# jacobwilliams/lbfgsb

Measured on NVIDIA B200. Metric: lbfgsb_iterations_per_s, higher is better.
Workload: dtype f64

## Files before the change

### lbfgsb_b200/csrc/engine.cu

```cuda
#include <cuda_runtime.h>
#include <dlfcn.h>
#include <stdarg.h>
#include <stdio.h>
#include <stdlib.h>
#include <string.h>

#include <mutex>
#include <string>
#include <unordered_set>
#include <vector>

#include "../../include/lbfgsb_b200.h"
#include "cauchy_walk.cuh"
#include "kernels_tma.cuh"
#include "cauchy_walk_dist.cuh"
#include "batch.cuh"
#include "host_print.h"
#include <algorithm>

static thread_local std::string g_last_error;
static void set_error(const char* fmt, ...) {
    char buf[512];
    va_list ap;
    va_start(ap, fmt);
// ... 199 lines not shown
        for (int q = 0; q < F_COUNT; ++q) { fam_ms[q] = 0; fam_calls[q] = 0; }
        if (st) stream = st;
        else { CK(cudaStreamCreateWithFlags(&stream, cudaStreamNonBlocking)); own_stream = true; }
        memset(&w, 0, sizeof w);
        w.n = n; w.m = m; w.off = offset;
        w.ldw = (n + 31) / 32 * 32;
        const size_t vb = (size_t)w.ldw * sizeof(T);
        if (!dalloc(&w.ws, vb * m) || !dalloc(&w.wy, vb * m)) return false;
        if (!dalloc(&w.z, vb) || !dalloc(&w.r, vb) || !dalloc(&w.d, vb) || !dalloc(&w.t, vb) || !dalloc(&w.xp, vb) || !dalloc(&w.gold, vb)) return false;
        if (!dalloc(&w.iwhere, (size_t)w.ldw * 4) || !dalloc(&w.state, (size_t)w.ldw)) return false;
        if (!dalloc(&w.part, sizeof(T) * LB_KMAX * LBFGSB_GRID) || !dalloc(&w.ipart, sizeof(i64) * LB_IMAX * LBFGSB_GRID)) return false;
        if (!dalloc(&w.part2, sizeof(T) * LB_KMAX * LBFGSB_GRID) || !dalloc(&w.ipart2, sizeof(i64) * LB_IMAX * LBFGSB_GRID)) return false;
        if (!dalloc(&s_dev, sizeof(DevState<T>)) || !dalloc(&pub_counter, 8) || !dalloc(&f_dev, sizeof(T))) return false;
        CK(cudaMemsetAsync(s_dev, 0, sizeof(DevState<T>), stream));
        CK(cudaMemsetAsync(pub_counter, 0, 8, stream));
        {
            i64 lim = (i64)1 << 28;
            if (R > 1) lim = (i64)1 << 26;
            if (const char* e = getenv("LBFGSB_B200_TIE_LIMIT")) lim = atoll(e);
            CK(cudaMemcpyAsync(&s_dev->tie_limit, &lim, sizeof lim, cudaMemcpyHostToDevice, stream));
        }
        CK(cudaMemsetAsync(w.ws, 0, vb * m, stream));
        CK(cudaMemsetAsync(w.wy, 0, vb * m, stream));
        w.s = s_dev;
        CK(cudaHostAlloc((void**)&s_host, sizeof(DevState<T>) + 64, cudaHostAllocMapped));
        memset(s_host, 0, sizeof(DevState<T>) + 64);
        pub_flag = (volatile unsigned long long*)((char*)s_host + ((sizeof(DevState<T>) + 7) / 8) * 8);
        CK(cudaMallocHost((void**)&ctl_host, sizeof(SortCtl)));
        header_bytes = offsetof(DevState<T>, sy);
        const i64 tile = (i64)LBFGSB_BLOCK * Real<T>::VEC * Real<T>::UNROLL;
        ntiles = (n + tile - 1) / tile;
        if (!dalloc(&tile_counts, sizeof(int) * (size_t)(ntiles + 1)) || !dalloc(&tile_offsets, sizeof(i64) * (size_t)(ntiles + 1))) return false;
        if (!dalloc(&rs_counts, sizeof(int) * 256 * LB_RS_GRID)) return false;
        typedef typename Real<T>::key_t K;
        memset(&wb, 0, sizeof wb);
        if (!dalloc(&wb.k0, sizeof(K) * (size_t)w.ldw) || !dalloc(&wb.k1, sizeof(K) * (size_t)w.ldw)) return false;
        if (!dalloc(&wb.v0, 4 * (size_t)w.ldw) || !dalloc(&wb.v1, 4 * (size_t)w.ldw)) return false;
        if (!dalloc(&wb.ctl, sizeof(SortCtl)) || !dalloc(&ctl_el, sizeof(SortCtl))) return false;
        i64 cap = n < (i64)(1 << 22) ? n : (i64)(1 << 22);
        cap = (cap + LB_WB - 1) / LB_WB * LB_WB;
        wb.cap = cap;
        const size_t cb = (size_t)cap * sizeof(T);
        if (!dalloc(&wb.wj, cb * 2 * m) || !dalloc(&wb.vj, cb * 2 * m)) return false;
        if (!dalloc(&wb.delta, cb) || !dalloc(&wb.zeta, cb) || !dalloc(&wb.omega, cb) || !dalloc(&wb.g2, cb) ||
            !dalloc(&wb.g1, cb) || !dalloc(&wb.f1a, cb) || !dalloc(&wb.f2a, cb)) return false;
        const i64 nblk = cap / LB_WB;
// ... 863 lines not shown
        i64 my_tie_limit = 0;
        if (ok && !write) ok = cudaMemcpy(&my_tie_limit, &s_dev->tie_limit, sizeof my_tie_limit, cudaMemcpyDeviceToHost) == cudaSuccess;
        const size_t CH = (size_t)64 << 20;
        void* stage = nullptr;
        if (ok && cudaMallocHost(&stage, CH) != cudaSuccess) { set_error("cudaMallocHost failed"); ok = false; }
        auto xfer = [&](void* dptr, size_t bytes) {
            for (size_t o = 0; ok && o < bytes; o += CH) {
                const size_t c = bytes - o < CH ? bytes - o : CH;
                if (write) {
                    ok = cudaMemcpy(stage, (char*)dptr + o, c, cudaMemcpyDeviceToHost) == cudaSuccess && fwrite(stage, 1, c, fp) == c;
                } else {
                    ok = fread(stage, 1, c, fp) == c && cudaMemcpy((char*)dptr + o, stage, c, cudaMemcpyHostToDevice) == cudaSuccess;
                }
            }
        };
        const size_t vb = (size_t)w.ldw * sizeof(T);
        xfer(s_dev, sizeof(DevState<T>));
        xfer(w.ws, vb * m); xfer(w.wy, vb * m);
        xfer(w.z, vb); xfer(w.r, vb); xfer(w.d, vb); xfer(w.t, vb); xfer(w.xp, vb); xfer(w.gold, vb);
        xfer(w.iwhere, (size_t)w.ldw * 4); xfer(w.state, (size_t)w.ldw);
        if (stage) cudaFreeHost(stage);
        if (ok && !write) ok = cudaMemcpy(&s_dev->tie_limit, &my_tie_limit, sizeof my_tie_limit, cudaMemcpyHostToDevice) == cudaSuccess;
        if (ok && !write) ok = cudaMemcpy(s_host, s_dev, header_bytes, cudaMemcpyDeviceToHost) == cudaSuccess;
        if (ok && !write) started = true;
        if (write && ok) ok = fflush(fp) == 0;
        if (fclose(fp) != 0) ok = false;
        if (write) {
            if (ok) ok = rename(tmp.c_str(), path) == 0;
            else remove(tmp.c_str());
        }
        if (!ok && g_last_error.empty()) set_error("checkpoint %s failed on %s", write ? "write" : "read", path);
        return ok;
    }

    bool active_hash(uint64_t* hash, i64* count) {
        begin(F_HASH); k_active_hash<T><<<LG>>>(w, offset); end(F_HASH);
        std::vector<i64> hp(2 * LBFGSB_GRID);
        CK(cudaMemcpyAsync(hp.data(), w.ipart, sizeof(i64) * 2 * LBFGSB_GRID, cudaMemcpyDeviceToHost, stream));
        CK(cudaStreamSynchronize(stream));
        uint64_t h = 0; i64 c = 0;
        for (int b = 0; b < LBFGSB_GRID; ++b) { h += (uint64_t)hp[b]; c += hp[LBFGSB_GRID + b]; }
        *hash = h; *count = c;
        return true;
    }
};

// ... 944 lines not shown
    if (!nccl_api()->ok) { set_error("libnccl.so.2 not found"); return nullptr; }
    ncclComm_t c = nullptr;
    ncclUniqueId id;
    memcpy(&id, id128, sizeof id);
    int rc = nccl_api()->CommInitRank(&c, world, id, rank);
    if (rc != 0) { set_error("ncclCommInitRank failed: %d", rc); return nullptr; }
    return c;
}
void lbfgsb_dev_nccl_destroy(void* comm) { if (comm && nccl_api()->ok) nccl_api()->CommDestroy((ncclComm_t)comm); }

int lbfgsb_dev_active_set_hash(lbfgsb_dev_t* h, uint64_t* hash, int64_t* count) {
    EngineBase* b = (EngineBase*)h;
    if (!b) return 1;
    i64 c = 0;
    bool ok = (b->real_kind == 8) ? ((Engine<double>*)b)->active_hash(hash, &c) : ((Engine<float>*)b)->active_hash(hash, &c);
    *count = c;
    return ok ? 0 : 1;
}
void* lbfgsb_dev_vector(lbfgsb_dev_t* h, int32_t which) {
    EngineBase* b = (EngineBase*)h;
    if (!b) return nullptr;
#define VSEL(E)                                                                                          \
    switch (which) { case 0: return E->w.z; case 1: return E->w.r; case 2: return E->w.d; case 3: return E->w.t; \
                     case 4: return E->w.xp; case 5: return E->w.ws; case 6: return E->w.wy; case 7: return E->w.iwhere; case 8: return E->w.gold; default: return nullptr; }
    if (b->real_kind == 8) { Engine<double>* e = (Engine<double>*)b; VSEL(e) }
    else { Engine<float>* e = (Engine<float>*)b; VSEL(e) }
}
int lbfgsb_dev_vector_copy(lbfgsb_dev_t* h, int32_t which, void* dst_dev, int64_t bytes) {
    void* src = lbfgsb_dev_vector(h, which);
    if (!src || !dst_dev || bytes < 0) return 1;
    EngineBase* b = (EngineBase*)h;
    const i64 ldw = (b->real_kind == 8) ? ((Engine<double>*)b)->w.ldw : ((Engine<float>*)b)->w.ldw;
    const i64 m = (b->real_kind == 8) ? ((Engine<double>*)b)->w.m : ((Engine<float>*)b)->w.m;
    const i64 cap = (which == 7) ? ldw * 4 : ((which == 5 || which == 6) ? m : 1) * ldw * (i64)b->real_kind;
    if (bytes > cap) { set_error("lbfgsb_dev_vector_copy: %lld bytes requested, vector %d holds %lld", (long long)bytes, (int)which, (long long)cap); return 1; }
    if (cudaDeviceSynchronize() != cudaSuccess) return 1;
    return cudaMemcpy(dst_dev, src, (size_t)bytes, cudaMemcpyDeviceToDevice) != cudaSuccess;
}
int lbfgsb_dev_exchange_mode(lbfgsb_dev_t* h) {
    EngineBase* b = (EngineBase*)h;
    if (!b) return -1;
    if (b->real_kind == 8) { Engine<double>* e = (Engine<double>*)b; return e->R <= 1 ? 0 : (e->p2p ? 2 : 1); }
    Engine<float>* e = (Engine<float>*)b; return e->R <= 1 ? 0 : (e->p2p ? 2 : 1);
}
int lbfgsb_dev_counters(lbfgsb_dev_t* h, int64_t* launches, int64_t* syncs) {
    EngineBase* b = (EngineBase*)h;
    if (!b) return 1;
    if (b->real_kind == 8) { *launches = ((Engine<double>*)b)->launches; *syncs = ((Engine<double>*)b)->syncs; }
    else { *launches = ((Engine<float>*)b)->launches; *syncs = ((Engine<float>*)b)->syncs; }
    return 0;
}
void lbfgsb_dev_profile(lbfgsb_dev_t* h, int32_t enable) {
    EngineBase* b = (EngineBase*)h;
    if (!b) return;
    if (b->real_kind == 8) ((Engine<double>*)b)->profile = enable != 0; else ((Engine<float>*)b)->profile = enable != 0;
}
void lbfgsb_dev_set_tie_limit(lbfgsb_dev_t* h, int64_t max_breakpoints) {
// ... 321 lines not shown
```

### lbfgsb_b200/csrc/kernels_dense.cuh

```cuda
#pragma once
#include "kernels_stream.cuh"

#define LB_SCALAR_THREADS 256

template <typename T>
struct Red {
    T rv[LB_KMAX];
    i64 iv[LB_IMAX];
};

enum { OP_SUM = 0, OP_MAX = 1, OP_MIN = 2, OP_ARGMIN = 3  };

struct SiteSpec {
    int nreal;
    int nint;
    int argmin_slot;
    int max_from, max_to;
    int min_from, min_to;
    int imin_from, imin_to;
    int imax_from, imax_to;
    int buf;
};

template <typename T>
// ... 348 lines not shown
        if (s->nbreak != 0 && !(s->dtm < s->bkmin)) {
            s->need_walk = 1; s->lazy_gcp = 0;
            for (int j = 0; j < col2; ++j) { s->p0[j] = s->p[j]; s->walkA[j] = zero; s->walkB[j] = zero; }
            s->walk_f1 = s->f1; s->walk_f2 = s->f2; s->walk_tlast = zero; s->walk_tprev2 = zero;
            s->walk_J = -1; s->walk_done = 0; s->walk_base = 0; s->walk_rcount = 0; s->walk_lcount = 0; s->walk_rem = 0;
            s->walk_cstart = 0; s->walk_fixn = 0; s->walk_closed = 0; s->tie_redo = 0; s->tie_round = 0;
            stop = 1;
        } else {
            if (s->dtm <= zero) s->dtm = zero;
            s->tsum = s->tsum + s->dtm;
            if (col > 0) dense::daxpy<T>(col2, s->dtm, s->p, s->c);
        }
    }
    stop = __shfl_sync(LB_FULL, stop, 0);
    if (stop) return;
    __syncwarp();
    if (fused_supported && col > 0 && s->cnstnd) {
        const int info = wdense::bmv<T>(m, ssy, swt, col, s->c, s->a);
        if (info == 0 && lane == 0) s->fuse_gf = 1;
    }
    __syncwarp();
}

template <typename T> __device__ inline void w_freev(DevState<T>* s, const Red<T>& red, i64 n_global, bool gf, bool have) {
    const int lane = threadIdx.x & 31;
    int need_a = 0;
    if (lane == 0) {
        if (s->fuse_gf == 1) s->lazy_z = 1;
        if (have) {
            s->nintol = s->nintol + s->nseg;
            s->nfree = red.iv[0];
            s->nenter = red.iv[1];
            s->nleave = red.iv[2];
            s->wrk = (s->nleave > 0) || (s->nenter > 0) || s->updatd;
            s->nact = n_global - s->nfree;
        }
        s->do_subspace = !(s->nfree == 0 || s->col == 0);
        s->do_formk = s->do_subspace && s->wrk;
        s->do_delta = s->do_formk && (s->nenter + s->nleave > 0);
        need_a = (!gf && s->do_subspace && !(!s->cnstnd && s->col > 0)) ? 1 : 0;
    }
    need_a = __shfl_sync(LB_FULL, need_a, 0);
    __syncwarp();
    if (need_a) {
        int info = wdense::bmv<T>(s->m, s->sy, s->wt, s->col, s->c, s->a);
        if (info != 0 && lane == 0) {
            ev_push<T>(s, EV_SUBSM_SINGULAR);
            reset_memory<T>(s);
            s->restart = 1; s->in_body = 0; s->do_subspace = 0; s->do_formk = 0; s->do_delta = 0;
        }
// ... 316 lines not shown
    if (!fused_supported || s->col <= 0 || !s->cnstnd || s->fuse_gf) return;
    stage_in<T>(ssy, s->sy, s->m * s->m); stage_in<T>(swt, s->wt, s->m * s->m);
    __syncthreads();
    if (threadIdx.x >= 32) return;
    const int info = wdense::bmv<T>(s->m, ssy, swt, s->col, s->c, s->a);
    if (info == 0 && (threadIdx.x & 31) == 0) s->fuse_gf = 2;
}

template <typename T>
__global__ void __launch_bounds__(LB_SCALAR_THREADS) s_freev(Wk<T> w, Dist<T> dist, i64 n_global, int phase) {
    __shared__ Red<T> red;
    DevState<T>* s = w.s;
    site_fetch<T>(w, dist);
    if (!s->go || !s->in_body) return;
    const bool gf = s->fuse_gf != 0;
    if (phase == 1 && !gf) return;
    if (phase == 0 && gf) {
        if (threadIdx.x == 0) { s->do_subspace = 1; s->do_formk = s->updatd; s->do_delta = 0; }
        return;
    }
    const int mode = s->cauchy_mode;
    if (mode != 1) site_reduce<T>(w, dist, site_freev(), &red);
    if (threadIdx.x >= 32) return;
    w_freev<T>(s, red, n_global, gf, mode != 1);
}

template <typename T>
__global__ void __launch_bounds__(LB_SCALAR_THREADS) s_formk_dense(Wk<T> w, Dist<T> dist, int mt, const T* delta, T* delta_sum) {
    __shared__ Red<T> red;
    DevState<T>* s = w.s;
    site_fetch<T>(w, dist);
    if (!s->go || !s->in_body || !s->do_subspace) return;
    const bool newrow = s->do_formk && s->updatd;
    if (newrow) site_reduce<T>(w, dist, site_formk(mt), &red);
    if (dist.R > 1 && s->do_delta) {
        if (dist.p2p) p2p_wait<T>(w, dist.p2p->dflag, dist.R, dist.dseq);
        const volatile T* dv = delta;
        for (int e = threadIdx.x; e < 6 * LB_MMAX * LB_MMAX; e += blockDim.x) {
            T acc = dv[e];
            for (int q = 1; q < dist.R; ++q) acc = acc + dv[(i64)q * (6 * LB_MMAX * LB_MMAX) + e];
            delta_sum[e] = acc;
        }
        __syncthreads();
        delta = delta_sum;
    }
    __shared__ T swn[4 * LB_MMAX * LB_MMAX], swn1[4 * LB_MMAX * LB_MMAX];
    const bool stage = s->do_formk != 0;
// ... 187 lines not shown
    if (upd) { stage_out<T>(s->sy, ssy, mm); stage_out<T>(s->ss, sss, mm); stage_out<T>(s->wt, swt, mm); }
    if (!cont) return;
    site_reduce<T>(w, dist, ms.sp[1], &red, ms.roff[1], ms.ioff[1]);
    if (threadIdx.x >= 32) return;
    w_cauchy<T>(s, red, mt, ssy, swt, 1);
    if (threadIdx.x != 0) return;
    if (!s->in_body) return;
    if (s->need_walk) { s->pause = PAUSE_WALK; return; }
    if (!s->fuse_gf) { s->pause = PAUSE_GCP_FREEV; return; }
    s->do_subspace = 1; s->do_formk = s->updatd; s->do_delta = 0;
}

template <typename T>
__global__ void __launch_bounds__(LB_SCALAR_THREADS) f_mid(Wk<T> w, Dist<T> dist, int mt, i64 n_global) {
    __shared__ Red<T> red;
    __shared__ T swn[4 * LB_MMAX * LB_MMAX], swn1[4 * LB_MMAX * LB_MMAX];
    __shared__ int cont;
    DevState<T>* s = w.s;
    const MSite ms = msite_mid(mt);
    site_fetch<T>(w, dist);
    if (!s->go || s->pause || !s->in_body) return;
    site_reduce<T>(w, dist, ms.sp[0], &red, ms.roff[0], ms.ioff[0]);
    if (threadIdx.x < 32) {
        w_freev<T>(s, red, n_global, true, true);
        if (threadIdx.x == 0) {
            cont = 1;
            if (!s->do_subspace) { s->pause = PAUSE_LSINIT; cont = 0; }
            else if (s->do_delta) { s->pause = PAUSE_DELTA; cont = 0; }
        }
    }
    __syncthreads();
    if (!cont) return;
    const bool newrow = s->do_formk && s->updatd;
    if (newrow) site_reduce<T>(w, dist, ms.sp[1], &red, ms.roff[1], ms.ioff[1]);
    const bool stage = s->do_formk != 0;
    const int m4 = 4 * s->m * s->m;
    stage_in<T>(swn, s->wn, m4);
    if (stage) stage_in<T>(swn1, s->wn1, m4);
    __syncthreads();
    if (threadIdx.x < 32) w_formk_dense<T>(s, red, mt, (const T*)nullptr, swn, swn1);
    __syncthreads();
    if (stage) { stage_out<T>(s->wn, swn, m4); stage_out<T>(s->wn1, swn1, m4); }
    if (!s->in_body) return;
    site_reduce<T>(w, dist, ms.sp[2], &red, ms.roff[2], ms.ioff[2]);
    if (threadIdx.x >= 32) return;
    w_subsm_dense<T>(s, red, mt, swn, 1);
}
// ... 22 lines not shown
```

### lbfgsb_b200/csrc/kernels_stream.cuh

```cuda
#pragma once
#include "common.cuh"

template <typename T>
struct Wk {
    i64 n, ldw;
    i64 off;
    int m;
    T *ws, *wy;
    T *z, *r, *d, *t, *xp;
    T* gold;
    int* iwhere;
    unsigned char* state;
    T* part;
    i64* ipart;
    T* part2;
    i64* ipart2;
    DevState<T>* s;
    T* x; const T* l; const T* u; const int* nbd; T* g;
    int bp_hint;
};

#define LB_SLOT(part, k) ((part) + (i64)(k) * LBFGSB_GRID)
#define LB_INF(T) ((T)INFINITY)
#define LB_I64MAX 0x7fffffffffffffffLL

template <typename T>
__global__ void __launch_bounds__(LBFGSB_BLOCK) k_errclb(Wk<T> w) {
    constexpr int VEC = Real<T>::VEC;
    i64 k6 = -1, k7 = -1;
    LB_FOR_TILES(T, w.n, base) {
        T l[VEC], u[VEC]; int nb[VEC];
        ldv<T>(w.l, base, w.n, l); ldv<T>(w.u, base, w.n, u); ldvi<T>(w.nbd, base, w.n, nb);
#pragma unroll
        for (int v = 0; v < VEC; ++v) {
            i64 i = base + v;
            if (i < w.n) {
                if (nb[v] < 0 || nb[v] > 3) k6 = i;
                if (nb[v] == 2 && l[v] > u[v]) k7 = i;
            }
        }
    }
    i64 m6 = k6, m7 = k7;
// ... 342 lines not shown
```

### lbfgsb_b200/csrc/kernels_tma.cuh

```cuda
#pragma once
#include "kernels_stream.cuh"
#include "tma_pipe.cuh"

template <typename T, int MT> struct SubT { static constexpr int v = (sizeof(T) * MT <= 80) ? 256 : 128; };

template <typename T> struct SpecializeFullHistory { static constexpr bool value = sizeof(T) == 4; };
template <bool B> struct BoolC { static constexpr bool value = B; };

#define LB_DYN_STAGES(dyn) (dyn)

template <typename T>
__device__ __forceinline__ void pipe_add_w(PipeSrc* ps, const Wk<T>& w, int head0, int count, unsigned slot) {
    int pj = head0;
    for (int j = 0; j < count; ++j) {
        pipe_add(ps, w.wy + (i64)pj * w.ldw, (int)sizeof(T), slot);
        pipe_add(ps, w.ws + (i64)pj * w.ldw, (int)sizeof(T), slot);
        pj = (pj + 1 == w.m) ? 0 : pj + 1;
    }
}

template <typename T, int MT>
__global__ void __launch_bounds__(LB_TMA_THREADS, 1) k_update(Wk<T> w) {
    constexpr int VEC = Real<T>::VEC;
    constexpr int SUBT = SubT<T, MT>::v;
// ... 480 lines not shown
                        ac[j] = ac[j] + wy[v] * dc[v];
                        ac[MT + j] = ac[MT + j] + wsv[v] * dc[v];
                    }
                }
            } else if (FULLC ? (j == MT - 1) : (j == col - 1)) {
#pragma unroll
                for (int v = 0; v < VEC; ++v)
                    if (mv[v]) {
                        ac[j] = ac[j] + y[v] * dc[v];
                        ac[MT + j] = ac[MT + j] + sn[v] * dc[v];
                    }
            }
        }
    });
    };
    if constexpr (SpecializeFullHistory<T>::value) { if (col == MT) pass(BoolC<true>{}); else pass(BoolC<false>{}); }
    else pass(BoolC<false>{});
    block_sum_store<T, 2 * MT + 1>(au, 2 * MT + 1, sm, w.part);
    block_sum_store<T, 2 * MT + 1>(ac, 2 * MT + 1, sm, w.part2);
    cauchy_scan_store<T, MT>(w, cs, smv, smi);
}
template <typename T, int MT> constexpr unsigned smem_update_classify() { return pipe_smem_bytes<T, SubT<T, MT>::v>(6 + 2 * (MT - 1), 2, 0); }

template <typename T, int MT, int GF>
__global__ void __launch_bounds__(LB_TMA_THREADS, 1) k_formk_cmprlb(Wk<T> w) {
    constexpr int VEC = Real<T>::VEC;
    constexpr int SUBT = SubT<T, MT>::v;
    typedef PipeGeom<T, SUBT> G;
    extern __shared__ __align__(128) char dyn[];
    __shared__ unsigned long long full[2 * LB_PIPE_STAGES];
    __shared__ PipeSrc ps;
    __shared__ T sm[4 * MT * (LBFGSB_BLOCK / 32)];
    __shared__ T coef[2 * MT];
    __shared__ i64 smi[LBFGSB_BLOCK / 32];
    const DevState<T>* s = w.s;
    if (!s->go || s->pause || !s->in_body || !s->do_subspace) return;
    constexpr bool gf = GF != 0;
    if (s->fuse_gf != GF) return;
    const bool gram = s->do_formk && s->updatd;
    const i64 n = w.n;
    const int col = s->col, head0 = s->head - 1;
    const T theta = s->theta;
    const bool uc = (!s->cnstnd && col > 0);
    const T tsum = s->tsum;
    const bool axpy = tsum != (T)0;
    const bool cnt = (s->iter > 0 && s->cnstnd);
    constexpr unsigned OG = 0, OX = G::REAL_SLOT, OZ = 2 * G::REAL_SLOT;
    constexpr unsigned OW = (GF == 1 ? 2u : 3u) * G::REAL_SLOT;
    if (threadIdx.x == 0) {
        pipe_begin(&ps);
        pipe_add(&ps, w.g, sizeof(T), G::REAL_SLOT);
        pipe_add(&ps, w.x, sizeof(T), G::REAL_SLOT);
        if (GF != 1) pipe_add(&ps, w.z, sizeof(T), G::REAL_SLOT);
        pipe_add_w<T>(&ps, w, head0, col, G::REAL_SLOT);
        pipe_add(&ps, w.state, 1, G::BYTE_SLOT);
        if (gf) pipe_add(&ps, w.iwhere, 4, G::INT_SLOT);
        pipe_end(&ps);
    }
    if (threadIdx.x < 2 * MT) {
        const int j = threadIdx.x % MT;
        coef[threadIdx.x] = (j < col) ? ((threadIdx.x < MT) ? s->a[j] : theta * s->a[col + j]) : (T)0;
    }
    T af[4 * MT], aw[2 * MT];
#pragma unroll
    for (int k = 0; k < 4 * MT; ++k) af[k] = (T)0;
#pragma unroll
    for (int k = 0; k < 2 * MT; ++k) aw[k] = (T)0;
    int nfr = 0, nen = 0, nle = 0;
    auto pass = [&](auto full_c) {
    constexpr bool FULLC = decltype(full_c)::value;
    const int colv = FULLC ? MT : col;
    const bool gramv = FULLC ? true : gram, ucv = FULLC ? false : uc;
    const unsigned ost = OW + 2u * (unsigned)colv * G::REAL_SLOT;
    const unsigned oiw = ost + G::BYTE_SLOT;
    const unsigned olast = OW + 2u * (unsigned)(colv - 1) * G::REAL_SLOT;
    tma_pass<T, SUBT>(n, &ps, LB_DYN_STAGES(dyn), full, [&](i64 base, const char* sb, int lt) {
        int st[VEC];
        lds_byte<T>(sb, ost, lt, st);
        bool fr[VEC]; bool any = false;
        T r[VEC];
        if (gf) {
            int iw[VEC];
            lds_int<T>(sb, oiw, lt, iw);
            T z[VEC], x[VEC], g[VEC];
            lds_real<T>(sb, OG, lt, g); lds_real<T>(sb, OX, lt, x);
            if (GF == 2) lds_real<T>(sb, OZ, lt, z);
#pragma unroll
            for (int v = 0; v < VEC; ++v) {
                const bool inr = base + v < n;
                const bool f = inr && iw[v] <= 0;
                const int old = st[v] & 1;
                nfr += f ? 1 : 0;
                if (cnt) { nen += (f && !old) ? 1 : 0; nle += (inr && !f && old) ? 1 : 0; }
                st[v] = (f ? 1 : 0) | ((cnt ? old : (f ? 1 : 0)) << 1) | ((iw[v] == 0 || iw[v] == -1) ? 4 : 0);
                fr[v] = f; any |= f;
                const T z0 = (GF == 2) ? z[v] : x[v];
                z[v] = axpy ? (z0 + tsum * cauchy_dir<T>(iw[v], g[v])) : z0;
                r[v] = ucv ? -g[v] : (-theta * (z[v] - x[v]) - g[v]);
            }
            stvb<T>(w.state, base, n, st);
            if (GF == 2 && axpy) stv<T>(w.z, base, n, z);
            if (!any && !gramv) return;
        } else {
#pragma unroll
            for (int v = 0; v < VEC; ++v) { fr[v] = (st[v] & 1) != 0; any |= fr[v]; }
            if (!any && !gramv) return;
// ... 54 lines not shown
        {
            T wyn[VEC], wsn[VEC];
            if (PREF) { lds_real_v<T>(sb, OW, lt, wyn); lds_real_v<T>(sb, OW + G::REAL_SLOT, lt, wsn); }
#pragma unroll
            for (int j = 0; j < MT; ++j) {
                if (j < col) {
                    T wy[VEC], wsv[VEC];
                    if (PREF) {
#pragma unroll
                        for (int v = 0; v < VEC; ++v) { wy[v] = wyn[v]; wsv[v] = wsn[v]; }
                        if (j + 1 < MT) {
                            lds_real_v<T>(sb, OW + (2 * j + 2) * G::REAL_SLOT, lt, wyn);
                            lds_real_v<T>(sb, OW + (2 * j + 3) * G::REAL_SLOT, lt, wsn);
                        }
                    } else {
                        lds_real<T>(sb, OW + (2 * j) * G::REAL_SLOT, lt, wy);
                        lds_real<T>(sb, OW + (2 * j + 1) * G::REAL_SLOT, lt, wsv);
                    }
#pragma unroll
                    for (int v = 0; v < VEC; ++v) {
                        const T py = wy[v] * r[v], psv = wsv[v] * r[v];
                        if (fr[v]) { aw[j] = aw[j] + py; aw[MT + j] = aw[MT + j] + psv; }
                    }
                }
            }
        }
        stv<T>(w.r, base, n, r);
    });
    };
    pass(BoolC<false>{});
    if (gram) block_sum_store<T, 4 * MT>(af, 4 * MT, sm, w.part);
    block_sum_store<T, 2 * MT>(aw, 2 * MT, sm, w.part2);
    if (gf) {
        i64 r0 = block_isum((i64)nfr, smi), r1 = block_isum((i64)nen, smi), r2 = block_isum((i64)nle, smi);
        if (threadIdx.x == 0) {
            LB_SLOT(w.ipart, 0)[blockIdx.x] = r0; LB_SLOT(w.ipart, 1)[blockIdx.x] = r1;
            LB_SLOT(w.ipart, 2)[blockIdx.x] = r2;
        }
    }
}
template <typename T, int MT> constexpr unsigned smem_formk_cmprlb() { return pipe_smem_bytes<T, SubT<T, MT>::v>(3 + 2 * MT, 1, 1); }

template <typename T, int MT, int PASS>
__global__ void __launch_bounds__(LB_TMA_THREADS, 1) k_subsm_lsinit(Wk<T> w) {
    constexpr int VEC = Real<T>::VEC;
    constexpr int SUBT = SubT<T, MT>::v;
    typedef PipeGeom<T, SUBT> G;
    extern __shared__ __align__(128) char dyn[];
    __shared__ unsigned long long full[2 * LB_PIPE_STAGES];
    __shared__ PipeSrc ps;
    __shared__ T sm[2 * (LBFGSB_BLOCK / 32)];
    __shared__ T smm[LBFGSB_BLOCK / 32];
    __shared__ i64 smi[LBFGSB_BLOCK / 32];
    const DevState<T>* s = w.s;
    if (!s->go || s->pause || !s->in_body || !s->do_subspace) return;
    const bool spec = s->spec_step != 0;
    if (PASS == 1 && !(spec && s->do_backtrack)) return;
    const i64 n = w.n;
    const int col = s->col, head0 = s->head - 1;
    const T theta = s->theta, rtheta = (T)1 / theta;
    const bool bounds = (s->cnstnd && s->iter != 0);
    const bool lz = s->lazy_z != 0;
    const T tsum = s->tsum;
    const bool axpy = tsum != (T)0;
    constexpr unsigned OX = 0, OG = G::REAL_SLOT, OL = 2 * G::REAL_SLOT, OU = 3 * G::REAL_SLOT, OR = 4 * G::REAL_SLOT,
                       OZ = 5 * G::REAL_SLOT;
    const unsigned OW = (lz ? 5u : 6u) * G::REAL_SLOT;
    if (threadIdx.x == 0) {
        pipe_begin(&ps);
        pipe_add(&ps, PASS == 1 ? w.t : w.x, sizeof(T), G::REAL_SLOT);
        pipe_add(&ps, w.g, sizeof(T), G::REAL_SLOT);
        pipe_add(&ps, w.l, sizeof(T), G::REAL_SLOT);
        pipe_add(&ps, w.u, sizeof(T), G::REAL_SLOT);
        pipe_add(&ps, w.r, sizeof(T), G::REAL_SLOT);
        if (!lz) pipe_add(&ps, w.z, sizeof(T), G::REAL_SLOT);
        pipe_add_w<T>(&ps, w, head0, col, G::REAL_SLOT);
        pipe_add(&ps, w.nbd, 4, G::INT_SLOT);
        pipe_add(&ps, w.state, 1, G::BYTE_SLOT);
        pipe_end(&ps);
    }
    T wv1[MT], wv2[MT];
#pragma unroll
    for (int j = 0; j < MT; ++j) { wv1[j] = (j < col) ? s->wv[j] : (T)0; wv2[j] = (j < col) ? s->wv[col + j] : (T)0; }
    T acc[2]; acc[0] = (T)0; acc[1] = (T)0;
    T smx = LB_INF(T);
    i64 iwd = 0;
    auto pass = [&](auto full_c) {
    constexpr bool FULLC = decltype(full_c)::value;
    const unsigned onb = OW + 2u * (unsigned)(FULLC ? MT : col) * G::REAL_SLOT, ost = onb + G::INT_SLOT;
    tma_pass<T, SUBT>(n, &ps, LB_DYN_STAGES(dyn), full, [&](i64 base, const char* sb, int lt) {
        int st[VEC];
        lds_byte<T>(sb, ost, lt, st);
        bool fr[VEC]; bool any = false;
#pragma unroll
        for (int v = 0; v < VEC; ++v) { fr[v] = (base + v < n) && (st[v] & 1); any |= fr[v]; }
        if (PASS == 1 && !any && !lz) return;
        T z[VEC], x[VEC], g[VEC];
        lds_real<T>(sb, OX, lt, x); lds_real<T>(sb, OG, lt, g);
        if (lz) {
#pragma unroll
            for (int v = 0; v < VEC; ++v) z[v] = axpy ? (x[v] + tsum * ((st[v] & 4) ? -g[v] : (T)0)) : x[v];
        } else lds_real<T>(sb, OZ, lt, z);
        T dk[VEC];
        if (any) {
            lds_real<T>(sb, OR, lt, dk);
#pragma unroll
            for (int j = 0; j < MT; ++j) {
                if (FULLC || j < col) {
                    T wy[VEC], wsv[VEC];
                    lds_real<T>(sb, OW + (2 * j) * G::REAL_SLOT, lt, wy);
                    lds_real<T>(sb, OW + (2 * j + 1) * G::REAL_SLOT, lt, wsv);
#pragma unroll
                    for (int v = 0; v < VEC; ++v) dk[v] = dk[v] + wy[v] * wv1[j] / theta + wsv[v] * wv2[j];
                }
            }
#pragma unroll
            for (int v = 0; v < VEC; ++v) dk[v] = rtheta * dk[v];
        }
        if (PASS == 1) {
            if (any) stv<T>(w.r, base, n, dk);
            if (lz) stv<T>(w.z, base, n, z);
            return;
        }
        T l[VEC], u[VEC]; int nb[VEC];
        lds_real<T>(sb, OL, lt, l); lds_real<T>(sb, OU, lt, u);
        lds_int<T>(sb, onb, lt, nb);
        if (!spec) stv<T>(w.xp, base, n, z);
        if (any) {
#pragma unroll
            for (int v = 0; v < VEC; ++v) {
                if (fr[v]) {
                    T xk = z[v];
                    if (nb[v] != 0) {
                        if (nb[v] == 1) { z[v] = dense::tmax(l[v], xk + dk[v]); if (z[v] == l[v]) iwd = 1; }
                        else if (nb[v] == 2) {
                            xk = dense::tmax(l[v], xk + dk[v]);
// ... 13 lines not shown
        for (int v = 0; v < VEC; ++v) {
            d[v] = z[v] - x[v];
            if (base + v < n) { acc[0] = acc[0] + d[v] * d[v]; acc[1] = acc[1] + d[v] * g[v]; }
        }
        stv<T>(w.d, base, n, d); stv<T>(w.t, base, n, x); stv<T>(w.gold, base, n, g);
        if (spec) stv<T>(w.x, base, n, z);
        if (bounds) {
#pragma unroll
            for (int v = 0; v < VEC; ++v) {
                if (base + v < n && nb[v] != 0) {
                    const T a1 = d[v];
                    if (a1 < (T)0 && nb[v] <= 2) {
                        const T a2 = l[v] - x[v];
                        const T cand = (a2 >= (T)0) ? (T)0 : a2 / a1;
                        smx = dense::tmin(smx, cand);
                    } else if (a1 > (T)0 && nb[v] >= 2) {
                        const T a2 = u[v] - x[v];
                        const T cand = (a2 <= (T)0) ? (T)0 : a2 / a1;
                        smx = dense::tmin(smx, cand);
                    }
                }
            }
        }
    });
    };
    if constexpr (SpecializeFullHistory<T>::value && PASS == 0) { if (col == MT) pass(BoolC<true>{}); else pass(BoolC<false>{}); }
    else pass(BoolC<false>{});
    if (PASS == 1) return;
    T ddp[1]; ddp[0] = acc[1];
    block_sum_store<T, 1>(ddp, 1, sm, w.part);
    i64 r0 = block_isum(iwd, smi);
    if (threadIdx.x == 0) LB_SLOT(w.ipart, 0)[blockIdx.x] = r0;
    block_sum_store<T, 2>(acc, 2, sm, w.part2);
    T rm = block_min<T>(smx, smm);
    if (threadIdx.x == 0) LB_SLOT(w.part2, 2)[blockIdx.x] = rm;
}
```

### lbfgsb_b200/csrc/tma_pipe.cuh

```cuda
#pragma once
#include "common.cuh"

namespace tma {

__device__ __forceinline__ unsigned smem_u32(const void* p) { return (unsigned)__cvta_generic_to_shared(p); }
__device__ __forceinline__ void mbar_init(unsigned long long* bar, int count) {
    asm volatile("mbarrier.init.shared::cta.b64 [%0], %1;" ::"r"(smem_u32(bar)), "r"(count) : "memory");
}
__device__ __forceinline__ void fence_barrier_init() { asm volatile("fence.mbarrier_init.release.cluster;" ::: "memory"); }
__device__ __forceinline__ void mbar_expect_tx(unsigned long long* bar, unsigned bytes) {
    asm volatile("mbarrier.arrive.expect_tx.shared::cta.b64 _, [%0], %1;" ::"r"(smem_u32(bar)), "r"(bytes) : "memory");
}
__device__ __forceinline__ void mbar_arrive(unsigned long long* bar) {
    asm volatile("mbarrier.arrive.shared::cta.b64 _, [%0];" ::"r"(smem_u32(bar)) : "memory");
}
__device__ __forceinline__ void mbar_wait(unsigned long long* bar, unsigned parity) {
    unsigned ok;
    do {
        asm volatile(
            "{\n"
            ".reg .pred p;\n"
            "mbarrier.try_wait.parity.shared::cta.b64 p, [%1], %2;\n"
            "selp.u32 %0, 1, 0, p;\n"
            "}\n"
// ... 65 lines not shown
    if (Real<T>::VEC == 2 && sizeof(T) == 4) {
        float a, b;
        asm volatile("ld.volatile.shared.v2.f32 {%0, %1}, [%2];" : "=f"(a), "=f"(b) : "r"(tma::smem_u32((const void*)e)));
        out[0] = (T)a; out[1] = (T)b;
    } else {
#pragma unroll
        for (int v = 0; v < Real<T>::VEC; ++v) out[v] = e[v];
    }
}
template <typename T>
__device__ __forceinline__ void lds_int(const char* sm, unsigned off, int lt, int (&out)[Real<T>::VEC]) {
    const typename Real<T>::ivec_t q = *reinterpret_cast<const typename Real<T>::ivec_t*>(sm + off + lt * (Real<T>::VEC * 4));
    const int* e = reinterpret_cast<const int*>(&q);
#pragma unroll
    for (int v = 0; v < Real<T>::VEC; ++v) out[v] = e[v];
}
template <typename T>
__device__ __forceinline__ void lds_byte(const char* sm, unsigned off, int lt, int (&out)[Real<T>::VEC]) {
    const unsigned char* b = reinterpret_cast<const unsigned char*>(sm + off + lt * Real<T>::VEC);
#pragma unroll
    for (int v = 0; v < Real<T>::VEC; ++v) out[v] = b[v];
}

#define LB_TMA_THREADS (LBFGSB_BLOCK + 32)

template <typename T, int SUBT, typename Body>
__device__ __forceinline__ void tma_pass(i64 n, const PipeSrc* ps, char* stages, unsigned long long* bars, Body body) {
    typedef PipeGeom<T, SUBT> G;
    constexpr int VEC = G::VEC;
    constexpr int NCW = LBFGSB_BLOCK / 32;
    const int tid = threadIdx.x, wid = tid >> 5, lane = tid & 31;
    unsigned long long* full = bars;
    unsigned long long* empty = bars + LB_PIPE_STAGES;
    const i64 tile = (i64)LBFGSB_BLOCK * VEC * Real<T>::UNROLL;
    const i64 ntiles = (n + tile - 1) / tile;
    const i64 b = blockIdx.x;
    i64 nitems = 0;
    if (ntiles > b) {
        const i64 ntl = (ntiles - b + LBFGSB_GRID - 1) / LBFGSB_GRID;
        const i64 tl_last = b + (ntl - 1) * LBFGSB_GRID;
        const i64 rem = n - tl_last * tile;
        i64 last = (rem + G::ELEMS - 1) / G::ELEMS;
        if (last > G::IPT) last = G::IPT;
        nitems = (ntl - 1) * G::IPT + last;
    }
    if (tid == 0) {
        for (int s = 0; s < LB_PIPE_STAGES; ++s) { tma::mbar_init(&full[s], 1); tma::mbar_init(&empty[s], NCW); }
        tma::fence_barrier_init();
    }
    __syncthreads();
    const unsigned stage_bytes = ps->stage_bytes;
    const int nsrc = ps->nsrc;
    auto stage_base = [&](i64 q) -> i64 {
        const i64 tl = b + (q / G::IPT) * LBFGSB_GRID;
        const int r = (int)(q % G::IPT);
        return tl * tile + (i64)r * G::ELEMS;
    };
    if (wid == NCW) {
        const unsigned stage_tx = ps->stage_tx;
        for (i64 q = 0; q < nitems; ++q) {
            const int st = (int)(q % LB_PIPE_STAGES);
            if (q >= LB_PIPE_STAGES) tma::mbar_wait(&empty[st], (unsigned)(((q / LB_PIPE_STAGES) - 1) & 1));
            const i64 sb = stage_base(q);
            if (sb + G::ELEMS <= n) {
                if (lane == 0) tma::mbar_expect_tx(&full[st], stage_tx);
                __syncwarp();
                char* dst = stages + (size_t)st * stage_bytes;
                for (int s = lane; s < nsrc; s += 32) {
                    const unsigned e = ps->esz[s];
                    tma::bulk_g2s(dst + ps->off[s], ps->p[s] + sb * e, (unsigned)G::ELEMS * e, &full[st]);
                }
            } else if (lane == 0) {
                tma::mbar_arrive(&full[st]);
            }
            __syncwarp();
        }
        return;
    }
    for (i64 q = 0; q < nitems; ++q) {
        const int st = (int)(q % LB_PIPE_STAGES);
        tma::mbar_wait(&full[st], (unsigned)((q / LB_PIPE_STAGES) & 1));
        const i64 sb = stage_base(q);
        const int h = (int)(q % G::HALVES);
        if (G::HALVES == 1 || tid / SUBT == h) {
            const int lt = tid % SUBT;
            char* sm = stages + (size_t)st * stage_bytes;
            const i64 base = sb + (i64)lt * VEC;
            if (sb + G::ELEMS > n) {
                for (int s = 0; s < nsrc; ++s) {
                    const unsigned e = ps->esz[s];
                    char* d = sm + ps->off[s] + (unsigned)lt * VEC * e;
                    const char* g = ps->p[s] + base * e;
                    for (unsigned v = 0; v < (unsigned)VEC; ++v)
                        for (unsigned c = 0; c < e; ++c) d[v * e + c] = (base + v < n) ? g[v * e + c] : (char)0;
                }
            }
            if (base < n) body(base, (const char*)sm, lt);
        }
        __syncwarp();
        if (lane == 0) tma::mbar_arrive(&empty[st]);
    }
}
```

Measured before the change: 93.71.

## Keep packed free-variable copies of W columns to shrink TMA loads in subspace pass

While forming K in the formk/cmprlb kernel, the free-variable rows of the WY/WS history are written into compacted per-512-element sub-tile buffers, with a per-tile free count. The later subspace pass reads those counts and TMA-loads only the packed prefix of each history column, rather than full dense slots. A producer-warp prep step with extra 'ready' mbarriers computes per-warp prefix offsets so consumers can index into the packed rows. This reduces global memory traffic when few variables are free, at the cost of extra device memory, extra scattered writes in formk, and more pipeline synchronization.

```diff
diff --git a/lbfgsb_b200/csrc/engine.cu b/lbfgsb_b200/csrc/engine.cu
--- a/lbfgsb_b200/csrc/engine.cu
+++ b/lbfgsb_b200/csrc/engine.cu
@@ -245,6 +245,19 @@
         }
         CK(cudaMemsetAsync(w.ws, 0, vb * m, stream));
         CK(cudaMemsetAsync(w.wy, 0, vb * m, stream));
+        if (!dalloc(&w.frow, sizeof(int))) return false;
+        CK(cudaMemsetAsync(w.frow, 0, sizeof(int), stream));
+        if (fused && R == 1) {
+            void *fs = nullptr, *fy = nullptr, *fc = nullptr;
+            if (cudaMalloc(&fs, vb * m) == cudaSuccess && cudaMalloc(&fy, vb * m) == cudaSuccess &&
+                cudaMalloc(&fc, sizeof(int) * (size_t)((w.ldw + 511) / 512)) == cudaSuccess) {
+                allocs.push_back(fs); allocs.push_back(fy); allocs.push_back(fc);
+                w.ws_f = (T*)fs; w.wy_f = (T*)fy; w.fcnt = (int*)fc;
+            } else {
+                cudaGetLastError();
+                for (void* q : {fs, fy, fc}) if (q) cudaFree(q);
+            }
+        }
         w.s = s_dev;
         CK(cudaHostAlloc((void**)&s_host, sizeof(DevState<T>) + 64, cudaHostAllocMapped));
         memset(s_host, 0, sizeof(DevState<T>) + 64);
@@ -1154,6 +1167,7 @@
         if (stage) cudaFreeHost(stage);
         if (ok && !write) ok = cudaMemcpy(&s_dev->tie_limit, &my_tie_limit, sizeof my_tie_limit, cudaMemcpyHostToDevice) == cudaSuccess;
         if (ok && !write) ok = cudaMemcpy(s_host, s_dev, header_bytes, cudaMemcpyDeviceToHost) == cudaSuccess;
+        if (ok && !write) ok = cudaMemset(w.frow, 0, sizeof(int)) == cudaSuccess;
         if (ok && !write) started = true;
         if (write && ok) ok = fflush(fp) == 0;
         if (fclose(fp) != 0) ok = false;
@@ -2144,7 +2158,9 @@
     if (!b) return nullptr;
 #define VSEL(E)                                                                                          \
     switch (which) { case 0: return E->w.z; case 1: return E->w.r; case 2: return E->w.d; case 3: return E->w.t; \
-                     case 4: return E->w.xp; case 5: return E->w.ws; case 6: return E->w.wy; case 7: return E->w.iwhere; case 8: return E->w.gold; default: return nullptr; }
+                     case 4: return E->w.xp; case 5: return E->w.ws; case 6: return E->w.wy; case 7: return E->w.iwhere; case 8: return E->w.gold; \
+                     case 9: return E->w.ws_f; case 10: return E->w.wy_f; case 11: return E->w.fcnt; case 12: return E->w.state; \
+                     case 13: return E->w.frow; default: return nullptr; }
     if (b->real_kind == 8) { Engine<double>* e = (Engine<double>*)b; VSEL(e) }
     else { Engine<float>* e = (Engine<float>*)b; VSEL(e) }
 }
@@ -2154,7 +2170,8 @@
     EngineBase* b = (EngineBase*)h;
     const i64 ldw = (b->real_kind == 8) ? ((Engine<double>*)b)->w.ldw : ((Engine<float>*)b)->w.ldw;
     const i64 m = (b->real_kind == 8) ? ((Engine<double>*)b)->w.m : ((Engine<float>*)b)->w.m;
-    const i64 cap = (which == 7) ? ldw * 4 : ((which == 5 || which == 6) ? m : 1) * ldw * (i64)b->real_kind;
+    const i64 cap = (which == 7) ? ldw * 4 : (which == 11) ? (ldw + 511) / 512 * 4 : (which == 12) ? ldw : (which == 13) ? 4 :
+                    ((which == 5 || which == 6 || which == 9 || which == 10) ? m : 1) * ldw * (i64)b->real_kind;
     if (bytes > cap) { set_error("lbfgsb_dev_vector_copy: %lld bytes requested, vector %d holds %lld", (long long)bytes, (int)which, (long long)cap); return 1; }
     if (cudaDeviceSynchronize() != cudaSuccess) return 1;
     return cudaMemcpy(dst_dev, src, (size_t)bytes, cudaMemcpyDeviceToDevice) != cudaSuccess;
diff --git a/lbfgsb_b200/csrc/kernels_dense.cuh b/lbfgsb_b200/csrc/kernels_dense.cuh
--- a/lbfgsb_b200/csrc/kernels_dense.cuh
+++ b/lbfgsb_b200/csrc/kernels_dense.cuh
@@ -394,10 +394,12 @@
     __syncwarp();
 }
 
-template <typename T> __device__ inline void w_freev(DevState<T>* s, const Red<T>& red, i64 n_global, bool gf, bool have) {
+template <typename T> __device__ inline void w_freev(DevState<T>* s, const Red<T>& red, i64 n_global, bool gf, bool have,
+                                                     int* frow = nullptr) {
     const int lane = threadIdx.x & 31;
     int need_a = 0;
     if (lane == 0) {
+        if (frow) *frow = gf ? 1 : 0;
         if (s->fuse_gf == 1) s->lazy_z = 1;
         if (have) {
             s->nintol = s->nintol + s->nseg;
@@ -760,7 +762,7 @@
     const int mode = s->cauchy_mode;
     if (mode != 1) site_reduce<T>(w, dist, site_freev(), &red);
     if (threadIdx.x >= 32) return;
-    w_freev<T>(s, red, n_global, gf, mode != 1);
+    w_freev<T>(s, red, n_global, gf, mode != 1, w.frow);
 }
 
 template <typename T>
@@ -994,7 +996,7 @@
     if (!s->go || s->pause || !s->in_body) return;
     site_reduce<T>(w, dist, ms.sp[0], &red, ms.roff[0], ms.ioff[0]);
     if (threadIdx.x < 32) {
-        w_freev<T>(s, red, n_global, true, true);
+        w_freev<T>(s, red, n_global, true, true, w.frow);
         if (threadIdx.x == 0) {
             cont = 1;
             if (!s->do_subspace) { s->pause = PAUSE_LSINIT; cont = 0; }
diff --git a/lbfgsb_b200/csrc/kernels_stream.cuh b/lbfgsb_b200/csrc/kernels_stream.cuh
--- a/lbfgsb_b200/csrc/kernels_stream.cuh
+++ b/lbfgsb_b200/csrc/kernels_stream.cuh
@@ -18,6 +18,9 @@
     DevState<T>* s;
     T* x; const T* l; const T* u; const int* nbd; T* g;
     int bp_hint;
+    T *ws_f, *wy_f;
+    int* fcnt;
+    int* frow;
 };
 
 #define LB_SLOT(part, k) ((part) + (i64)(k) * LBFGSB_GRID)
diff --git a/lbfgsb_b200/csrc/kernels_tma.cuh b/lbfgsb_b200/csrc/kernels_tma.cuh
--- a/lbfgsb_b200/csrc/kernels_tma.cuh
+++ b/lbfgsb_b200/csrc/kernels_tma.cuh
@@ -526,17 +526,65 @@
 }
 template <typename T, int MT> constexpr unsigned smem_update_classify() { return pipe_smem_bytes<T, SubT<T, MT>::v>(6 + 2 * (MT - 1), 2, 0); }
 
+#define LB_FROW_MAX (7 * 512 / 8)
+
+template <bool IW>
+__device__ __forceinline__ void frow_prep(const char* sm, unsigned ost, unsigned oiw, int c, int* info) {
+    const int lane = threadIdx.x & 31;
+    if (sm == nullptr || (!IW && c == LB_FROW_DENSE)) {
+        if (lane == 0) info[0] = LB_FROW_DENSE;
+        return;
+    }
+    const uint4 sq = *reinterpret_cast<const uint4*>(sm + ost + lane * 16);
+    const unsigned sw[4] = {sq.x & 0x01010101u, sq.y & 0x01010101u, sq.z & 0x01010101u, sq.w & 0x01010101u};
+    unsigned fb = 0;
+#pragma unroll
+    for (int k = 0; k < 4; ++k) fb |= ((sw[k] | (sw[k] >> 7) | (sw[k] >> 14) | (sw[k] >> 21)) & 0xfu) << (4 * k);
+    bool chg = false;
+    if (IW) {
+        const int4* iw = reinterpret_cast<const int4*>(sm + oiw) + lane * 4;
+        unsigned nb = 0;
+#pragma unroll
+        for (int k = 0; k < 4; ++k) {
+            const int4 a = iw[k];
+            nb |= ((unsigned)(a.x <= 0) | (unsigned)(a.y <= 0) << 1 | (unsigned)(a.z <= 0) << 2 | (unsigned)(a.w <= 0) << 3) << (4 * k);
+        }
+        chg = nb != fb;
+        fb = nb;
+    }
+    const int cnt = __popc(fb);
+    int incl = cnt;
+#pragma unroll
+    for (int o = 1; o < 32; o <<= 1) {
+        const int t = __shfl_up_sync(0xffffffffu, incl, o);
+        if (lane >= o) incl += t;
+    }
+    if ((lane & 3) == 0) info[2 + (lane >> 2)] = incl - cnt;
+    chg = __any_sync(0xffffffffu, chg);
+    if (lane == 31) {
+        info[0] = IW ? (incl <= LB_FROW_MAX ? incl : LB_FROW_DENSE) : c;
+        info[1] = chg ? 1 : 0;
+    }
+}
+__device__ __forceinline__ void frow_pos(const bool (&fr)[2], int lower, int (&pos)[2]) {
+    const unsigned lm = (1u << (threadIdx.x & 31)) - 1u;
+    const unsigned b0 = __ballot_sync(0xffffffffu, fr[0]), b1 = __ballot_sync(0xffffffffu, fr[1]);
+    pos[0] = lower + __popc(b0 & lm) + __popc(b1 & lm);
+    pos[1] = pos[0] + (fr[0] ? 1 : 0);
+}
+
 template <typename T, int MT, int GF>
 __global__ void __launch_bounds__(LB_TMA_THREADS, 1) k_formk_cmprlb(Wk<T> w) {
     constexpr int VEC = Real<T>::VEC;
     constexpr int SUBT = SubT<T, MT>::v;
     typedef PipeGeom<T, SUBT> G;
     extern __shared__ __align__(128) char dyn[];
-    __shared__ unsigned long long full[2 * LB_PIPE_STAGES];
+    __shared__ unsigned long long full[3 * LB_PIPE_STAGES];
     __shared__ PipeSrc ps;
     __shared__ T sm[4 * MT * (LBFGSB_BLOCK / 32)];
     __shared__ T coef[2 * MT];
     __shared__ i64 smi[LBFGSB_BLOCK / 32];
+    __shared__ int sinfo[LB_PIPE_STAGES * LB_PREP_INTS];
     const DevState<T>* s = w.s;
     if (!s->go || s->pause || !s->in_body || !s->do_subspace) return;
     constexpr bool gf = GF != 0;
@@ -549,6 +597,9 @@
     const T tsum = s->tsum;
     const bool axpy = tsum != (T)0;
     const bool cnt = (s->iter > 0 && s->cnstnd);
+    static_assert(!gf || (G::ELEMS == 512 && VEC == 2), "the free-row copy is laid out in 512-variable sub-tiles");
+    const bool keep = gf && w.fcnt != nullptr;
+    const bool add1 = keep && *w.frow != 0 && s->updatd;
     constexpr unsigned OG = 0, OX = G::REAL_SLOT, OZ = 2 * G::REAL_SLOT;
     constexpr unsigned OW = (GF == 1 ? 2u : 3u) * G::REAL_SLOT;
     if (threadIdx.x == 0) {
@@ -578,14 +629,25 @@
     const unsigned ost = OW + 2u * (unsigned)colv * G::REAL_SLOT;
     const unsigned oiw = ost + G::BYTE_SLOT;
     const unsigned olast = OW + 2u * (unsigned)(colv - 1) * G::REAL_SLOT;
-    tma_pass<T, SUBT>(n, &ps, LB_DYN_STAGES(dyn), full, [&](i64 base, const char* sb, int lt) {
+    auto body = [&](i64 base, const char* sb, int lt) {
         int st[VEC];
         lds_byte<T>(sb, ost, lt, st);
         bool fr[VEC]; bool any = false;
         T r[VEC];
+        constexpr int FROW_ALL = 1 << 11, FROW_BIAS = 1 << 10;
+        int fp = -1;
         if (gf) {
             int iw[VEC];
             lds_int<T>(sb, oiw, lt, iw);
+            if (keep) {
+                const int* inf = sinfo + (sb == LB_DYN_STAGES(dyn) ? 0 : LB_PREP_INTS);
+                if (inf[0] != LB_FROW_DENSE) {
+                    const bool f[VEC] = {iw[0] <= 0, iw[1] <= 0};
+                    int pos[VEC];
+                    frow_pos(f, inf[2 + (lt >> 5)], pos);
+                    fp = FROW_BIAS + pos[0] - lt * VEC + ((add1 && !inf[1]) ? 0 : FROW_ALL);
+                }
+            }
             T z[VEC], x[VEC], g[VEC];
             lds_real<T>(sb, OG, lt, g); lds_real<T>(sb, OX, lt, x);
             if (GF == 2) lds_real<T>(sb, OZ, lt, z);
@@ -686,11 +748,25 @@
                         const T py = wy[v] * r[v], psv = wsv[v] * r[v];
                         if (fr[v]) { aw[j] = aw[j] + py; aw[MT + j] = aw[MT + j] + psv; }
                     }
+                    if (gf && fp >= 0 && (fp >= FROW_ALL || j == col - 1)) {
+                        const i64 at = ((const T*)ps.p[OW / G::REAL_SLOT + 2 * j] - w.wy) + base + ((fp & (FROW_ALL - 1)) - FROW_BIAS);
+                        if (fr[0]) { w.wy_f[at] = wy[0]; w.ws_f[at] = wsv[0]; }
+                        if (fr[1]) { w.wy_f[at + fr[0]] = wy[1]; w.ws_f[at + fr[0]] = wsv[1]; }
+                    }
                 }
             }
         }
         stv<T>(w.r, base, n, r);
-    });
+    };
+    if constexpr (gf) {
+        auto prep = [&](const char* stage, i64 sb0, int c, int* info) {
+            if (!keep) return;
+            frow_prep<true>(stage, ost, oiw, c, info);
+            __syncwarp();
+            if ((threadIdx.x & 31) == 0) w.fcnt[sb0 / G::ELEMS] = info[0];
+        };
+        tma_pass<T, SUBT>(n, &ps, LB_DYN_STAGES(dyn), full, body, PipePacked{}, stage_prep(prep), sinfo);
+    } else tma_pass<T, SUBT>(n, &ps, LB_DYN_STAGES(dyn), full, body);
     };
     pass(BoolC<false>{});
     if (gram) block_sum_store<T, 4 * MT>(af, 4 * MT, sm, w.part);
@@ -711,8 +787,9 @@
     constexpr int SUBT = SubT<T, MT>::v;
     typedef PipeGeom<T, SUBT> G;
     extern __shared__ __align__(128) char dyn[];
-    __shared__ unsigned long long full[2 * LB_PIPE_STAGES];
+    __shared__ unsigned long long full[3 * LB_PIPE_STAGES];
     __shared__ PipeSrc ps;
+    __shared__ int sinfo[LB_PIPE_STAGES * LB_PREP_INTS];
     __shared__ T sm[2 * (LBFGSB_BLOCK / 32)];
     __shared__ T smm[LBFGSB_BLOCK / 32];
     __shared__ i64 smi[LBFGSB_BLOCK / 32];
@@ -743,6 +820,12 @@
         pipe_add(&ps, w.state, 1, G::BYTE_SLOT);
         pipe_end(&ps);
     }
+    const bool rd = PASS == 0 && w.fcnt != nullptr && *w.frow != 0;
+    PipePacked pk{};
+    if (rd) {
+        pk.cnt = w.fcnt; pk.fy = (const char*)w.wy_f; pk.fs = (const char*)w.ws_f; pk.slot_bytes = w.ldw * (i64)sizeof(T);
+        pk.w0 = lz ? 5 : 6; pk.nw = 2 * col; pk.head0 = head0; pk.m = s->m;
+    }
     T wv1[MT], wv2[MT];
 #pragma unroll
     for (int j = 0; j < MT; ++j) { wv1[j] = (j < col) ? s->wv[j] : (T)0; wv2[j] = (j < col) ? s->wv[col + j] : (T)0; }
@@ -752,13 +835,21 @@
     auto pass = [&](auto full_c) {
     constexpr bool FULLC = decltype(full_c)::value;
     const unsigned onb = OW + 2u * (unsigned)(FULLC ? MT : col) * G::REAL_SLOT, ost = onb + G::INT_SLOT;
-    tma_pass<T, SUBT>(n, &ps, LB_DYN_STAGES(dyn), full, [&](i64 base, const char* sb, int lt) {
+    auto body = [&](i64 base, const char* sb, int lt) {
         int st[VEC];
         lds_byte<T>(sb, ost, lt, st);
         bool fr[VEC]; bool any = false;
 #pragma unroll
         for (int v = 0; v < VEC; ++v) { fr[v] = (base + v < n) && (st[v] & 1); any |= fr[v]; }
         if (PASS == 1 && !any && !lz) return;
+        bool packed = false; int fpos[VEC];
+        if (rd) {
+            const int* inf = sinfo + (sb == LB_DYN_STAGES(dyn) ? 0 : LB_PREP_INTS);
+            if (inf[0] != LB_FROW_DENSE) {
+                packed = true;
+                frow_pos(fr, inf[2 + (lt >> 5)], fpos);
+            }
+        }
         T z[VEC], x[VEC], g[VEC];
         lds_real<T>(sb, OX, lt, x); lds_real<T>(sb, OG, lt, g);
         if (lz) {
@@ -768,14 +859,30 @@
         T dk[VEC];
         if (any) {
             lds_real<T>(sb, OR, lt, dk);
-#pragma unroll
-            for (int j = 0; j < MT; ++j) {
-                if (FULLC || j < col) {
-                    T wy[VEC], wsv[VEC];
-                    lds_real<T>(sb, OW + (2 * j) * G::REAL_SLOT, lt, wy);
-                    lds_real<T>(sb, OW + (2 * j + 1) * G::REAL_SLOT, lt, wsv);
-#pragma unroll
-                    for (int v = 0; v < VEC; ++v) dk[v] = dk[v] + wy[v] * wv1[j] / theta + wsv[v] * wv2[j];
+            if (packed) {
+#pragma unroll
+                for (int v = 0; v < VEC; ++v) {
+                    if (!fr[v]) continue;
+                    const char* pr = sb + OW + (unsigned)fpos[v] * (unsigned)sizeof(T);
+#pragma unroll
+                    for (int j = 0; j < MT; ++j) {
+                        if (FULLC || j < col) {
+                            const T wy = *reinterpret_cast<const T*>(pr + (2 * j) * G::REAL_SLOT);
+                            const T wsv = *reinterpret_cast<const T*>(pr + (2 * j + 1) * G::REAL_SLOT);
+                            dk[v] = dk[v] + wy * wv1[j] / theta + wsv * wv2[j];
+                        }
+                    }
+                }
+            } else {
+#pragma unroll
+                for (int j = 0; j < MT; ++j) {
+                    if (FULLC || j < col) {
+                        T wy[VEC], wsv[VEC];
+                        lds_real<T>(sb, OW + (2 * j) * G::REAL_SLOT, lt, wy);
+                        lds_real<T>(sb, OW + (2 * j + 1) * G::REAL_SLOT, lt, wsv);
+#pragma unroll
+                        for (int v = 0; v < VEC; ++v) dk[v] = dk[v] + wy[v] * wv1[j] / theta + wsv[v] * wv2[j];
+                    }
                 }
             }
 #pragma unroll
@@ -835,7 +942,11 @@
                 }
             }
         }
-    });
+    };
+    if constexpr (PASS == 0) {
+        auto prep = [&](const char* stage, i64, int c, int* info) { if (rd) frow_prep<false>(stage, ost, 0, c, info); };
+        tma_pass<T, SUBT>(n, &ps, LB_DYN_STAGES(dyn), full, body, pk, stage_prep(prep), sinfo);
+    } else tma_pass<T, SUBT>(n, &ps, LB_DYN_STAGES(dyn), full, body);
     };
     if constexpr (SpecializeFullHistory<T>::value && PASS == 0) { if (col == MT) pass(BoolC<true>{}); else pass(BoolC<false>{}); }
     else pass(BoolC<false>{});
diff --git a/lbfgsb_b200/csrc/tma_pipe.cuh b/lbfgsb_b200/csrc/tma_pipe.cuh
--- a/lbfgsb_b200/csrc/tma_pipe.cuh
+++ b/lbfgsb_b200/csrc/tma_pipe.cuh
@@ -111,16 +111,39 @@
     for (int v = 0; v < Real<T>::VEC; ++v) out[v] = b[v];
 }
 
+#define LB_FROW_DENSE (-1)
+
+struct PipePacked {
+    const int* cnt;
+    const char *fy, *fs;
+    i64 slot_bytes;
+    int w0, nw, head0, m;
+};
+
+struct NoPrep {
+    static constexpr bool on = false;
+    __device__ void operator()(const char*, i64, int, int*) const {}
+};
+template <typename F> struct StagePrep {
+    static constexpr bool on = true;
+    F f;
+    __device__ __forceinline__ void operator()(const char* sm, i64 sb, int c, int* info) const { f(sm, sb, c, info); }
+};
+template <typename F> __device__ __forceinline__ StagePrep<F> stage_prep(F f) { return StagePrep<F>{f}; }
+#define LB_PREP_INTS 10
+
 #define LB_TMA_THREADS (LBFGSB_BLOCK + 32)
 
-template <typename T, int SUBT, typename Body>
-__device__ __forceinline__ void tma_pass(i64 n, const PipeSrc* ps, char* stages, unsigned long long* bars, Body body) {
+template <typename T, int SUBT, typename Body, typename Prep = NoPrep>
+__device__ __forceinline__ void tma_pass(i64 n, const PipeSrc* ps, char* stages, unsigned long long* bars, Body body,
+                                         const PipePacked& pk = PipePacked{}, Prep prep = Prep{}, int* info = nullptr) {
     typedef PipeGeom<T, SUBT> G;
     constexpr int VEC = G::VEC;
     constexpr int NCW = LBFGSB_BLOCK / 32;
     const int tid = threadIdx.x, wid = tid >> 5, lane = tid & 31;
     unsigned long long* full = bars;
     unsigned long long* empty = bars + LB_PIPE_STAGES;
+    unsigned long long* ready = bars + 2 * LB_PIPE_STAGES;
     const i64 tile = (i64)LBFGSB_BLOCK * VEC * Real<T>::UNROLL;
     const i64 ntiles = (n + tile - 1) / tile;
     const i64 b = blockIdx.x;
@@ -134,7 +157,10 @@
         nitems = (ntl - 1) * G::IPT + last;
     }
     if (tid == 0) {
-        for (int s = 0; s < LB_PIPE_STAGES; ++s) { tma::mbar_init(&full[s], 1); tma::mbar_init(&empty[s], NCW); }
+        for (int s = 0; s < LB_PIPE_STAGES; ++s) {
+            tma::mbar_init(&full[s], 1); tma::mbar_init(&empty[s], NCW);
+            if (Prep::on) tma::mbar_init(&ready[s], 1);
+        }
         tma::fence_barrier_init();
     }
     __syncthreads();
@@ -147,27 +173,53 @@
     };
     if (wid == NCW) {
         const unsigned stage_tx = ps->stage_tx;
+        int cnext = (pk.cnt && nitems > 0) ? pk.cnt[stage_base(0) / G::ELEMS] : LB_FROW_DENSE;
+        int cprev = LB_FROW_DENSE;
+        auto prep_stage = [&](i64 p, int c) {
+            const int st = (int)(p % LB_PIPE_STAGES);
+            tma::mbar_wait(&full[st], (unsigned)((p / LB_PIPE_STAGES) & 1));
+            const i64 sb = stage_base(p);
+            prep(sb + G::ELEMS <= n ? stages + (size_t)st * stage_bytes : nullptr, sb, c, info + st * LB_PREP_INTS);
+            __syncwarp();
+            if (lane == 0) tma::mbar_arrive(&ready[st]);
+        };
         for (i64 q = 0; q < nitems; ++q) {
             const int st = (int)(q % LB_PIPE_STAGES);
+            if (Prep::on && q > 0) prep_stage(q - 1, cprev);
+            const int c = cnext;
+            if (pk.cnt && q + 1 < nitems) cnext = pk.cnt[stage_base(q + 1) / G::ELEMS];
             if (q >= LB_PIPE_STAGES) tma::mbar_wait(&empty[st], (unsigned)(((q / LB_PIPE_STAGES) - 1) & 1));
             const i64 sb = stage_base(q);
             if (sb + G::ELEMS <= n) {
-                if (lane == 0) tma::mbar_expect_tx(&full[st], stage_tx);
+                const unsigned pb = (c == LB_FROW_DENSE) ? G::REAL_SLOT : (((unsigned)c * (unsigned)sizeof(T) + 15u) & ~15u);
+                if (lane == 0) tma::mbar_expect_tx(&full[st], stage_tx - (unsigned)pk.nw * (G::REAL_SLOT - pb));
                 __syncwarp();
                 char* dst = stages + (size_t)st * stage_bytes;
                 for (int s = lane; s < nsrc; s += 32) {
                     const unsigned e = ps->esz[s];
+                    const unsigned k = (unsigned)(s - pk.w0);
+                    if (c != LB_FROW_DENSE && k < (unsigned)pk.nw) {
+                        if (pb == 0) continue;
+                        int pj = pk.head0 + (int)(k >> 1);
+                        if (pj >= pk.m) pj -= pk.m;
+                        const char* src = ((k & 1) ? pk.fs : pk.fy) + (i64)pj * pk.slot_bytes + sb * (i64)sizeof(T);
+                        tma::bulk_g2s(dst + ps->off[s], src, pb, &full[st]);
+                        continue;
+                    }
                     tma::bulk_g2s(dst + ps->off[s], ps->p[s] + sb * e, (unsigned)G::ELEMS * e, &full[st]);
                 }
             } else if (lane == 0) {
                 tma::mbar_arrive(&full[st]);
             }
             __syncwarp();
+            cprev = c;
         }
+        if (Prep::on && nitems > 0) prep_stage(nitems - 1, cprev);
         return;
     }
     for (i64 q = 0; q < nitems; ++q) {
         const int st = (int)(q % LB_PIPE_STAGES);
+        if (Prep::on) tma::mbar_wait(&ready[st], (unsigned)((q / LB_PIPE_STAGES) & 1));
         tma::mbar_wait(&full[st], (unsigned)((q / LB_PIPE_STAGES) & 1));
         const i64 sb = stage_base(q);
         const int h = (int)(q % G::HALVES);
```

New measurement: 92.15 (median of 6 runs). 0.983x the previous value.
